# tsurumeso/vocal-remover

Measured on AMD Instinct MI355X. Metric: spectrogram-frames/sec (inference, CascadedNet n_fft=2048), higher is better.
Workload: dtype f32; 1 GPU; configs[1]: 30 s stereo 44.1 kHz synthetic song, STFT -> 11 crops of 256 frames in one device batch -> predict_mask -> stitch -> mask apply -> iSTFT x2; n_fft=2048, hop=1024, cropsize=256, parallelism=replicas x1 (songs shard, no collective), input_residency=inputs resident in HBM when the timed region starts

## Files before the change

__graft_entry__.py:

```python
import concurrent.futures
import importlib.util
import os
import subprocess
import sys

ROOT = os.path.dirname(os.path.abspath(__file__))
PKG_DIR = os.path.join(ROOT, 'vocal-remover_amd')
CSRC = os.path.join(PKG_DIR, 'csrc')
LIB = os.path.join(PKG_DIR, 'libvr_mi355.so')
SOURCES = ['conv_mfma.hip', 'conv_ws.hip', 'conv_dma.hip', 'conv_wino.hip', 'conv_x3.hip', 'conv_x3h.hip', 'conv_x3d.hip', 'conv_x3s.hip', 'conv_thin.hip', 'wgrad_mfma.hip', 'wgrad_wino.hip', 'wgrad_gemm.hip', 'pointwise.hip', 'backward.hip', 'lstm.hip', 'stft.hip', 'augment.hip', 'audio.hip', 'model.hip',
           'train.hip', 'debug.hip', 'comm.hip', 'profile.hip', 'api.cpp', 'pcm_host.cpp']
HEADERS = sorted(f for f in os.listdir(CSRC) if f.endswith('.h')) + [os.path.join('..', '..', 'include', 'vr_mi355.h')]
HIPCC = os.environ.get('HIPCC', '/opt/rocm/bin/hipcc')
FLAGS = ['--offload-arch=gfx950', '-O3', '-std=c++17', '-fPIC', '-Wno-unused-result', '-Rpass-analysis=kernel-resource-usage']
MAX_SCRATCH_BYTES_PER_LANE = 192
ZERO_SCRATCH_KERNELS = ('conv_x3_kernel', 'conv_x3h_kernel', 'conv_x3d_kernel', 'conv_x3d_aspp_kernel', 'wgrad_wino_r_kernel')


def _newer(target, deps):
    if not os.path.exists(target):
        return True
    t = os.path.getmtime(target)
    return any(os.path.getmtime(d) > t for d in deps)


def _compile(src):
    path = os.path.join(CSRC, src)
    obj = os.path.join(CSRC, os.path.splitext(src)[0] + '.o')
    deps = [path] + [os.path.join(CSRC, h) for h in HEADERS]
    if _newer(obj, deps):
        cmd = [HIPCC] + FLAGS + (['-x', 'hip'] if src.endswith('.cpp') else []) + ['-c', path, '-o', obj]
        r = subprocess.run(cmd, capture_output=True, text=True)
        if r.returncode != 0:
# ... 66 lines not shown
```

vocal-remover_amd/csrc/conv_x3d.hip:

```cpp
#include <cstdlib>
#include <type_traits>

#include "conv_epilogue.h"
#include "conv_stage.h"
#include "kernels.h"
#include "lds_dma.h"
#include "x3h_common.h"

namespace vr {

template <int KK, int DH, int DW, int MT, int TH>
struct X3dCfg {
    static_assert(KK == 9 || KK == 1, "3x3 or 1x1");
    static constexpr int TW = 16, CK = 8;
    static constexpr int HH = KK == 9 ? DH : 0, HW = KK == 9 ? DW : 0;
    static constexpr int TH_in = TH + 2 * HH, PW = TW + 2 * HW;
    static constexpr int NSLOT = TH_in * PW;
    static constexpr int NREAL = TH_in * TW;
    static constexpr int NPASS = (NREAL + 255) / 256;
    static constexpr int WM = MT / 32, WN = TH / 8;
    static constexpr int PLANE = NSLOT * 16, P_BYTES = 2 * PLANE;
    static constexpr int NWP = KK * 2 * MT, W_BYTES = NWP * 16, NWPASS = (NWP + 255) / 256;
    static constexpr int E_OFF = P_BYTES + 2 * W_BYTES;
    static constexpr int M_OFF = E_OFF + 4 * MT * 4;
// ... 336 lines not shown
                a.part[((long long)pt * a.Cout + co) * 2 + 1] = s2;
            }
        }
    }
}

__device__ __forceinline__ bool x3d_block(const ConvArgs& a, int& pt, int& ct) {
    const int id = blockIdx.x;
    const int xcd = id & 7, rr = id >> 3;
    ct = rr % a.nct;
    const int per_xcd = (a.npt + 7) >> 3;
    pt = xcd * per_xcd + rr / a.nct;
    return pt < a.npt;
}

template <int KK, int DH, int DW, int MT>
__global__ __launch_bounds__(256, 2) void conv_x3d_kernel(const ConvArgs a) {
    extern __shared__ __attribute__((aligned(16))) char smem_x3d[];
    int pt, ct;
    if (!x3d_block(a, pt, ct)) return;
    x3d_tile<KK, DH, DW, MT, 16>(a, pt, ct, smem_x3d);
}

struct X3dAsppArgs { ConvArgs c[4]; };
template <int MT>
__global__ __launch_bounds__(256, 2) void conv_x3d_aspp_kernel(const X3dAsppArgs g) {
    extern __shared__ __attribute__((aligned(16))) char smem_x3d[];
    int pt, ct;
    if (!x3d_block(g.c[1], pt, ct)) return;
    if (blockIdx.y == 0) x3d_tile<9, 12, 6, MT, 16>(g.c[3], pt, ct, smem_x3d);
    else if (blockIdx.y == 1) x3d_tile<9, 8, 4, MT, 16>(g.c[2], pt, ct, smem_x3d);
    else if (blockIdx.y == 2) x3d_tile<9, 4, 2, MT, 16>(g.c[1], pt, ct, smem_x3d);
    else x3d_tile<1, 1, 1, MT, 16>(g.c[0], pt, ct, smem_x3d);
}

bool x3d_pick(const ConvArgs& a, const ConvShape& s, int* MT_out) {
    static const int enabled = getenv("VR_CONV_X3D") ? atoi(getenv("VR_CONV_X3D")) : 1;
    if (!enabled || a.bf16 != 3 || !a.x3w || a.tapmask) return false;
    if (s.stride != 1 || a.Win != 16 || a.Wout != 16 || a.Hin != a.Hout) return false;
    if (s.KS == 3) {
        const bool dil = (s.dil_h == 1 && s.dil_w == 1) || (s.dil_h == 4 && s.dil_w == 2) || (s.dil_h == 8 && s.dil_w == 4) ||
                         (s.dil_h == 12 && s.dil_w == 6);
        if (!dil || a.pad_h != s.dil_h || a.pad_w != s.dil_w) return false;
    } else if (s.KS == 1) {
        if (a.pad_h != 0 || a.pad_w != 0) return false;
    } else return false;
    for (int i = 0; i < a.nsrc; ++i) {
        const ConvSrc& c = a.src[i];
        if (c.aff0 || c.aff1 || c.post || c.zins || c.up || c.slope != 1.f || c.W != 16 || c.H != a.Hin) return false;
        if ((long long)c.H * (c.sH > 0 ? c.sH : 1) * 4 >= 0x7FFFFFF0LL) return false;
    }
    static const int force_mt = getenv("VR_X3D_MT") ? atoi(getenv("VR_X3D_MT")) : 0;
// ... 20 lines not shown
    VR_HIP(hipGetLastError());
}
template <int MT>
static void x3d_launch_mt(const ConvArgs& a, const ConvShape& s, hipStream_t st) {
    if (s.KS == 1) x3d_launch<1, 1, 1, MT>(a, st);
    else if (s.dil_h == 1) x3d_launch<9, 1, 1, MT>(a, st);
    else if (s.dil_h == 4) x3d_launch<9, 4, 2, MT>(a, st);
    else if (s.dil_h == 8) x3d_launch<9, 8, 4, MT>(a, st);
    else x3d_launch<9, 12, 6, MT>(a, st);
}
void x3d_launch_conv(const ConvArgs& a, const ConvShape& s, int MT, hipStream_t st) {
    if (MT == 64) x3d_launch_mt<64>(a, s, st);
    else x3d_launch_mt<32>(a, s, st);
}

template <int MT>
static void x3d_launch_aspp_mt(const X3dAsppArgs& g, hipStream_t st) {
    auto kern = conv_x3d_aspp_kernel<MT>;
    constexpr int lds = X3dCfg<9, 12, 6, MT, 16>::LDS_BYTES;
    static_assert(lds >= X3dCfg<9, 8, 4, MT, 16>::LDS_BYTES && lds >= X3dCfg<1, 1, 1, MT, 16>::LDS_BYTES, "the widest halo sizes the LDS");
    static std::atomic<unsigned long long> attr_done{0};
    ensure_lds_attr(attr_done, reinterpret_cast<const void*>(kern), lds);
    const ConvArgs& a = g.c[1];
    VR_LAUNCH(kern, dim3((unsigned)((a.npt + 7) / 8 * 8 * a.nct), 4u), dim3(256), lds, st, g);
    VR_HIP(hipGetLastError());
}
bool x3d_aspp_eligible(const ConvArgs* c, const ConvShape* s) {
    static const bool on = !(getenv("VR_ASPP_FUSED") && atoi(getenv("VR_ASPP_FUSED")) == 0);
    if (!on) return false;
    int mt[4];
    for (int j = 0; j < 4; ++j) {
        if (!x3d_pick(c[j], s[j], &mt[j])) return false;
        if (c[j].N != c[0].N || c[j].Hout != c[0].Hout || c[j].CoutPad != c[0].CoutPad) return false;
    }
    return s[0].KS == 1 && s[1].KS == 3 && s[1].dil_h == 4 && s[2].KS == 3 && s[2].dil_h == 8 && s[3].KS == 3 && s[3].dil_h == 12;
}
void x3d_launch_aspp(const ConvArgs* c, hipStream_t st) {
    X3dAsppArgs g;
    int MT = (c[1].CoutPad % 64 == 0) ? 64 : 32;
    if (MT == 64 && (long long)c[1].N * ((c[1].Hout + 15) / 16) * (c[1].CoutPad / 64) * 4 < 512) MT = 32;
    static const int force_mt = getenv("VR_X3D_MT") ? atoi(getenv("VR_X3D_MT")) : 0;
    if ((force_mt == 32 || force_mt == 64) && c[1].CoutPad % force_mt == 0) MT = force_mt;
    for (int j = 0; j < 4; ++j) { g.c[j] = c[j]; x3d_fill_tiling(g.c[j], MT); }
    if (MT == 64) x3d_launch_aspp_mt<64>(g, st);
    else x3d_launch_aspp_mt<32>(g, st);
}

}
```

vocal-remover_amd/csrc/debug.hip:

```cpp
#include <cmath>
#include <cstdlib>
#include <cstring>
#include <memory>
#include <string>
#include <vector>

#include "model.h"

namespace vr {

namespace {

struct DevBuf {
    float* p = nullptr;
    size_t n = 0;
    DevBuf() = default;
    explicit DevBuf(size_t n_) : n(n_) {
        VR_HIP(hipMalloc(&p, (n ? n : 1) * sizeof(float)));
        VR_HIP(hipMemset(p, 0, (n ? n : 1) * sizeof(float)));
        VR_HIP(hipStreamSynchronize(nullptr));
    }
    DevBuf(const float* host, size_t n_) : n(n_) {
        VR_HIP(hipMalloc(&p, (n ? n : 1) * sizeof(float)));
        if (host && n) VR_HIP(hipMemcpy(p, host, n * sizeof(float), hipMemcpyHostToDevice));
// ... 914 lines not shown
        need(5, 0, 2, 1);
        const long long rows = dims[0];
        const int T = (int)dims[1], Wm = (int)dims[2], off = (int)dims[3];
        const bool cplx = dims[4] != 0;
        VR_CHECK(rows > 0 && Wm > 0 && off >= 0 && off + Wm <= T, -2, "crop: need rows, Wm > 0 and 0 <= off, off + Wm <= T");
        const bool loss = !cplx && nin >= 3 && in[2] && nout >= 2 && out[1];
        const size_t E = cplx ? 2 : 1;
        DevBuf m(in[0], (size_t)rows * Wm * E), x(in[1], (size_t)rows * T * E), y(loss ? in[2] : nullptr, loss ? (size_t)rows * T : 0);
        DevBuf part((size_t)l1_crop_blocks()), lossd(4);
        launch_mul_crop(x.p, m.p, cplx, rows, T, Wm, off, st);
        if (loss) launch_l1_crop(L1_CROP_REAL, m.p, y.p, rows, T, Wm, off, part.p, lossd.p, st);
        VR_HIP(hipStreamSynchronize(st));
        m.download(out[0]);
        if (loss) VR_HIP(hipMemcpy(out[1], lossd.p, sizeof(float), hipMemcpyDeviceToHost));
    } else if (name == "rows") {
        need(3, 0, 3, 2);
        const int N = (int)dims[0], R = (int)dims[1], W = (int)dims[2];
        const size_t n = (size_t)N * R * W;
        DevBuf x(in[0], n), aff(in[1], (size_t)R * 2), d(in[2], n), o(n), sums(R);
        launch_rows_affine_relu(x.p, o.p, aff.p, N, R, W, st);
        launch_channel_sum(d.p, N, R, W, sums.p, 0, st);
        VR_HIP(hipStreamSynchronize(st));
        o.download(out[0]); sums.download(out[1]);
    } else if (name == "adam") {
        need(1, 6, 4, 3);
        const size_t n = (size_t)dims[0];
        double dp[6];
        for (int i = 0; i < 6; ++i) {
            char buf[48];
            std::snprintf(buf, sizeof buf, "%.7g", (double)fp[i]);
            dp[i] = std::strtod(buf, nullptr);
        }
        DevBuf p(in[0], n), g(in[1], n), m(in[2], n), v(in[3], n);
        launch_adam(p.p, g.p, m.p, v.p, (long long)n, dp[0], dp[1], dp[2], dp[3], (long long)dp[5], dp[4], st);
        VR_HIP(hipStreamSynchronize(st));
        p.download(out[0]); m.download(out[1]); v.download(out[2]);
    } else if (name == "wire") {
        need(1, 0, 1, 1);
        const size_t n = (size_t)dims[0];
        DevBuf x(in[0], n), half((n + 1) / 2), y(n);
        launch_f32_to_bf16(x.p, reinterpret_cast<unsigned short*>(half.p), (long long)n, st);
        launch_bf16_to_f32(reinterpret_cast<const unsigned short*>(half.p), y.p, (long long)n, st);
        VR_HIP(hipStreamSynchronize(st));
        y.download(out[0]);
    } else if (name == "signal_norm") {
        need(6, 0, 1, 2);
// ... 222 lines not shown
```

vocal-remover_amd/csrc/kernels.h:

```cpp
#pragma once
#include "vr_common.h"

namespace vr {

struct HeadDst {
    float* p;
    long long dN, dC, dH;
    int w_lo, w_hi;
    int pad_rows;
    float* const* items;
    const int* item_pitch;
};
void launch_head_sigmoid(const Tensor& x, const float* w , const HeadDst& d, hipStream_t st);
void launch_head_complex(const Tensor& x, const float* w , const HeadDst& d, hipStream_t st);
int launch_squeeze_conv(const Tensor& x, const float* w , float* out, float* part, bool dry, hipStream_t st,
                        const float* epi = nullptr);

void launch_avgpool_h(const Tensor& x, float* out, hipStream_t st);

struct BNFoldDesc { const float *w, *b, *rm, *rv; float* affine; int C; int bcast; };
void launch_bn_fold_eval(const BNFoldDesc* d_descs, int ndesc, int maxC, float eps, hipStream_t st);
struct BNFinalizeArgs {
    const float* part; int nparts; int pstride;
    double count;
// ... 25 lines not shown
void launch_wino_weights(const float* w, float* u, int Cin, int CoutPad, hipStream_t st);
struct WinoWDesc { const float* w; void* u; int Cin, CoutPad; };
void launch_wino_weights_batched(const WinoWDesc* d_descs, int n, long long max_elems, bool split6, hipStream_t st);
size_t wino_weights6_bytes(int Cin, int CoutPad);
void launch_wino_weights6(const float* w, void* u6, int Cin, int CoutPad, hipStream_t st);
struct X3Tile { int MT, TH; };
struct X3WDesc { const float* w; void* o; int Cin, KK, CoutPad; };
bool x3_pick(const ConvArgs& a, const ConvShape& s, X3Tile* t);
void x3_fill_tiling(ConvArgs& a, const X3Tile& t);
void x3_launch_conv(const ConvArgs& a, const X3Tile& t, hipStream_t st);
size_t x3_weights_bytes(int Cin, int KK, int CoutPad);
void launch_x3_weights(const float* w, void* o, int Cin, int KK, int CoutPad, hipStream_t st);
void launch_x3_weights_batched(const X3WDesc* d_descs, int n, long long max_elems, hipStream_t st);
void x3h_launch_conv(const ConvArgs& a, const X3Tile& t, hipStream_t st);
bool x3h_tail_ok(const ConvArgs& a, const X3Tile& t);
void x3h_trace_read(long long* host, int n);
void x3h_trace_clear();
void launch_x3h_weights(const float* w, void* o, int Cin, int KK, int CoutPad, hipStream_t st);
void launch_x3h_weights_batched(const X3WDesc* d_descs, int n, long long max_elems, int max_cout_pad, hipStream_t st);
bool x3d_pick(const ConvArgs& a, const ConvShape& s, int* MT);
void x3d_fill_tiling(ConvArgs& a, int MT);
void x3d_launch_conv(const ConvArgs& a, const ConvShape& s, int MT, hipStream_t st);
bool x3d_aspp_eligible(const ConvArgs* c4, const ConvShape* s4);
void x3d_launch_aspp(const ConvArgs* c4, hipStream_t st);
bool x3s_pick(const ConvArgs& a, const ConvShape& s, X3Tile* t);
void x3s_fill_tiling(ConvArgs& a, const X3Tile& t);
void x3s_launch_conv(const ConvArgs& a, const X3Tile& t, hipStream_t st);
void launch_upsample2x(const Tensor& x, float* out, hipStream_t st);

void launch_bilstm(const float* gx, const float* whh_f, const float* whh_r, float* out,
                   int N, int T, int H, hipStream_t st);

void launch_bilstm_train(const float* gx, const float* whh_f, const float* whh_r, float* out, float* save,
                         int N, int T, int H, hipStream_t st);
void launch_bilstm_bwd(const float* dh, const float* save, const float* whh_f, const float* whh_r, float* dgx,
                       int N, int T, int H, hipStream_t st);
size_t lstm_whh_grad_scratch_floats(int N, int H);
void launch_lstm_whh_grad(const float* dgx, const float* hout, float* dwhh_f, float* dwhh_r, int N, int T, int H,
                          int accumulate, float* part, hipStream_t st);

struct BnBwdArgs {
    float* g;
    const float* z;
    int N, C, H, W;
    long long sN, sC, sH;
    const float* aff;
    int aff_bcast;
    float slope;
    const float* post;
    const float *gamma, *save_mean, *save_invstd;
    float *dgamma, *dbeta;
    int acc_grads;
    float* coef;
    float* part;
};
int bn_bwd_chunks(const BnBwdArgs& a);
void launch_bn_bwd(const BnBwdArgs& a, hipStream_t st);

void launch_upsample_bwd(const float* dhi, int N, int C, int H, int W, float* glo, long long gN, long long gC,
                         long long gH, int accumulate, hipStream_t st);
void launch_sum_h(const float* d, int N, int C, int H, int W, float* out, hipStream_t st);
void launch_avgpool_bwd(const float* gp, float* g, int N, int C, int H, int W, long long sN, long long sC, long long sH,
// ... 197 lines not shown
```

vocal-remover_amd/csrc/model.h:

```cpp
#pragma once
#include <chrono>
#include <deque>
#include <functional>
#include <map>
#include <memory>
#include <string>
#include <vector>

#include "kernels.h"
#include "weight_forms.h"

namespace vr {

struct Arena {
    char* base = nullptr;
    size_t cap = 0, off = 0, peak = 0;
    bool dry = false;
    void* alloc(size_t bytes) {
        const size_t a = (off + 255) & ~size_t(255);
        off = a + bytes;
        if (off > peak) peak = off;
        if (dry) return reinterpret_cast<void*>(uintptr_t(256));
        if (off > cap) throw Error(-4, "workspace arena overflow (planning bug)");
        return base + a;
// ... 223 lines not shown
    void debug_weight_forms(const float* dw_kmajor, int Cin, int KS, int stride, int dh, int dw, int CoutPad, int Win, bool transformed,
                            ConvArgs& a, LocalConv& lc);
    bool record_taps = false;
    std::map<std::string, Tensor> taps;
    int64_t get_tap(const std::string& name, float* host, int64_t cap_floats, int64_t* shape4);

    bool profiling = false;
    LaunchProfiler* launch_prof = nullptr;
    std::string profile_report;
    void profile_begin();
    void augment_api(const float* Xc, const float* yc, const float* Xi, const float* yi, const void* desc, const float* rw,
                     int B, int T, int bins, bool in_on_dev, float* Xmag, float* ymag, bool out_on_dev, bool out_complex = false);
    void dataset_batch_api(const ResidentSet& set, const ResidentCrop* crops, const void* desc, const float* rw, int B, int T,
                           float* Xmag, float* ymag, bool out_on_dev, bool out_complex = false);
    char* aug_buf = nullptr; size_t aug_cap = 0;
    void aug_reserve(size_t need);
    bool train_wino = true;
    int mfma_mode = 3;
    bool x3_mode() const { return mfma_mode == 2 || mfma_mode == 3; }
    int default_mfma_mode = 3;
    bool serial = false;
    bool crop_window = true;
    bool fuse_tail = true;
    int net_w_lo = 0, net_w_hi = 0;
    void set_option(const std::string& name, int value);
    void reset_adam_state();
    void profile_end(double* conv_ms, double* conv_flops, double* conv_bytes, int* launches);

    hipStream_t stream = nullptr;
    hipStream_t side_stream = nullptr;
    hipEvent_t ev_fork = nullptr, ev_join = nullptr;
    bool band_fork_active = false;
    bool gs_clear_pending = false;
    bool wgrad_on_side = false;
    struct Lane { hipStream_t main = nullptr, side = nullptr; hipEvent_t fork = nullptr, join = nullptr, start = nullptr, done = nullptr; Arena ws; };
    std::vector<Lane> lanes;
    void swap_lane(int i);

private:
    float* p_arena = nullptr; size_t p_floats = 0;
    float* b_arena = nullptr; size_t b_floats = 0;
    Arena ws;
    Arena io;
    void ensure_ws(size_t bytes);
    int plan_B = -1, plan_T = -1; bool plan_training = false; size_t plan_peak = 0;
    void ensure_io(size_t bytes);
// ... 154 lines not shown
```

vocal-remover_amd/csrc/model.hip:

```cpp
#include "pcm.h"
#include "model.h"

#include <algorithm>
#include <chrono>
#include <cmath>
#include <cstdlib>
#include <cstring>

namespace vr {

static inline int round_up(int v, int m) { return (v + m - 1) / m * m; }

Param* Model::add_param(const std::string& key, std::vector<int64_t> shape, ParamKind kind, bool trainable) {
    params.emplace_back();
    Param* p = &params.back();
    p->key = key;
    p->shape = std::move(shape);
    p->kind = kind;
    p->trainable = trainable;
    p->numel = 1;
    for (auto d : p->shape) p->numel *= (size_t)d;
    p->dev_numel = p->numel;
    if (kind == PK_CONV) {
        p->Cout = (int)p->shape[0];
// ... 314 lines not shown
    affine_dirty = false;
}

void Model::set_option(const std::string& name, int value) {
    plan_peak = 0;
    if (name == "train_winograd") train_wino = value != 0;
    else if (name == "serial_exec") serial = value != 0;
    else if (name == "params_dirty") affine_dirty = true;
    else if (name == "mfma_bf16") { mfma_mode = value != 0 ? 1 : default_mfma_mode; affine_dirty = true; }
    else if (name == "mfma_mode") {
        if (value < -1 || value > 3) throw Error(-2, "mfma_mode: 0, 1, 2, 3 or -1 (default)");
        mfma_mode = value < 0 ? default_mfma_mode : value; affine_dirty = true;
    }
    else if (name == "conv_x3d") {
        if (value < -1 || value > 2) throw Error(-2, "conv_x3d: 0, 1, 2 or -1 (default)");
        x3d_mode = value < 0 ? 2 : value;
    }
    else if (name == "conv_x3s") {
        if (value < -1 || value > 1) throw Error(-2, "conv_x3s: 0, 1 or -1 (default)");
        x3s_mode = value < 0 ? x3s_default() : value;
    }
    else if (name == "crop_window") crop_window = value != 0;
    else if (name == "fuse_tail") fuse_tail = value != 0;
    else if (name == "complex_train") {
        if (!is_complex) throw Error(-2, "complex_train: this handle predicts a magnitude mask; the option belongs to complex-mask handles (VR_CREATE_COMPLEX)");
        complex_train = value != 0;
        if (!complex_train && loss_kind != 0) set_loss(0, 0.01);
        graph_valid = false;
    }
    else if (name == "adam_reset") reset_adam_state();
    else if (name == "hip_graph" || name == "conv_x3p" || name == "wgrad_x3h" || name == "conv_x3b") {
        static std::string told;
        if (told.find("|" + name + "|") == std::string::npos) {
            told += "|" + name + "|";
            fprintf(stderr, "libvr_mi355: option '%s' was retired with its kernel (tools/experiments/README.md); ignored\n", name.c_str());
        }
    }
    else throw Error(-2, "unknown option: " + name);
}

void Model::hold_form(FormId f, const std::vector<Conv*>& convs, Wino6Want w6, FormStore& s) {
    if (s.arena[f]) return;
    auto room = [&](const Conv* L) {
        const FormSpec sp = form_spec(f, *L, mfma_mode, w6);
        return sp.held ? (sp.bytes + 255) & ~size_t(255) : size_t(0);
    };
// ... 458 lines not shown
            b->nbt->nbt += 1;
        }
    }
    Tensor zt;
    zt.p = z; zt.N = N; zt.C = nb; zt.H = 1; zt.W = nf;
    zt.sN = (long long)nb * nf; zt.sC = nf; zt.sH = nf;
    if (training) { zt.aff0 = M.squeeze.bn->affine; zt.slope = 0.f; }
    else zt.slope = 1.f;
    if (taping()) {
        zt.g = galloc((size_t)N * nb * nf, false);
        TapeRec r;
        r.kind = TK_SQUEEZE; r.M = &M; r.srcs = {SrcSpec{h}}; r.N = N;
        r.out = zt;
        r.out.C = 1; r.out.H = nb; r.out.sC = (long long)nb * nf; r.out.sH = nf;
        tape.push_back(std::move(r));
    }
    const int G = 4 * M.hid;
    float* bias = ws.allocf((size_t)2 * G);
    if (!training && M.bias_sum) bias = M.bias_sum;
    else if (!dry) {
        launch_add(M.b_ih_f->dev, M.b_hh_f->dev, bias, G, stream);
        launch_add(M.b_ih_r->dev, M.b_hh_r->dev, bias + G, G, stream);
    }
    Tensor gx = run_conv(M.proj, {SrcSpec{zt}}, N, nullptr, bias, true);
    float* hc = ws.allocf((size_t)N * 2 * M.hid * nf);
    float* save = taping() ? ws.allocf((size_t)N * 2 * nf * 5 * M.hid) : nullptr;
    if (!dry) launch_bilstm_train(gx.p, M.whh_f->dev, M.whh_r->dev, hc, save, N, nf, M.hid, stream);
    Tensor ht;
    ht.p = hc; ht.N = N; ht.C = 2 * M.hid; ht.H = 1; ht.W = nf;
    ht.sN = (long long)2 * M.hid * nf; ht.sC = nf; ht.sH = nf; ht.slope = 1.f;
    if (taping()) {
        ht.g = galloc((size_t)N * 2 * M.hid * nf, false);
        TapeRec r;
        r.kind = TK_LSTM; r.M = &M; r.N = N; r.out = ht; r.aux = gx; r.save = save;
        tape.push_back(std::move(r));
    }
    Tensor lin = run_conv(M.dense, {SrcSpec{ht}}, N, nullptr, M.dense_b->dev, true);
    if (taping()) tape.back().bias_param = M.dense_b;
    float* act = training ? ws.allocf((size_t)N * nb * nf) : lin.p;
    if (!dry && training) launch_rows_affine_relu(lin.p, act, M.dense.bn->affine, N, nb, nf, stream);
    Tensor o;
    o.p = act; o.g = lin.g; o.N = N; o.C = 1; o.H = nb; o.W = nf;
    o.sN = (long long)nb * nf; o.sC = (long long)nb * nf; o.sH = nf; o.slope = 1.f;
    return o;
}

Model::SrcSpec Model::upsampled(const Tensor& t) {
    if (training) {
        SrcSpec s{t};
        s.up = true;
        return s;
    }
    static const bool fuse_on = !(getenv("VR_X3_FUSE_UP") && atoi(getenv("VR_X3_FUSE_UP")) == 0);
    static const bool x3_on = !(getenv("VR_CONV_X3") && atoi(getenv("VR_CONV_X3")) == 0);
    if (fuse_on && x3_on && x3_mode() && 4LL * t.H * t.W >= 65536 && 2 * t.W >= 32 && !t.aff0 && !t.aff1 && !t.post && t.slope == 1.f) {
        SrcSpec s{t};
        s.up = true;
        return s;
    }
    Tensor u;
    u.N = t.N; u.C = t.C; u.H = 2 * t.H; u.W = 2 * t.W;
    u.sH = u.W; u.sC = (long long)u.H * u.W; u.sN = u.sC * u.C; u.slope = 1.f;
    u.p = ws.allocf((size_t)u.N * u.C * u.H * u.W);
    if (!dry) launch_upsample2x(t, u.p, stream);
    return SrcSpec{u};
}

Tensor Model::run_basenet(BaseNetL& B, const std::vector<SrcSpec>& in, int N, const Tensor* out_view, FusedTail* tail) {
    const std::string& p = B.prefix;
    Tensor e[5];
    e[0] = run_conv(B.enc1, in, N, nullptr, nullptr, false);
    tap(p + ".e1", e[0]);
    for (int i = 0; i < 4; ++i) {
        Tensor t = run_conv(B.enc_a[i], {SrcSpec{e[i]}}, N, nullptr, nullptr, false);
        e[i + 1] = run_conv(B.enc_b[i], {SrcSpec{t}}, N, nullptr, nullptr, false);
        tap(p + ".e" + std::to_string(i + 2), e[i + 1]);
    }
    const Tensor& x5 = e[4];
    const int C8 = 8 * B.c;
    float* pooled = ws.allocf((size_t)N * C8 * x5.W);
    if (!dry) launch_avgpool_h(x5, pooled, stream);
    Tensor pt;
    pt.p = pooled; pt.N = N; pt.C = C8; pt.H = 1; pt.W = x5.W;
    pt.sN = (long long)C8 * x5.W; pt.sC = x5.W; pt.sH = x5.W; pt.slope = 1.f;
    if (taping()) {
        pt.g = galloc((size_t)N * C8 * x5.W, false);
        TapeRec r;
        r.kind = TK_AVGPOOL; r.srcs = {SrcSpec{x5}}; r.out = pt; r.N = N;
        tape.push_back(std::move(r));
    }
    Tensor f1 = run_conv(B.aspp_pool, {SrcSpec{pt}}, N, nullptr, nullptr, true);
    Tensor cat4;
    cat4.N = N; cat4.C = 4 * C8; cat4.H = x5.H; cat4.W = x5.W;
    cat4.sH = x5.W; cat4.sC = (long long)x5.H * x5.W; cat4.sN = cat4.sC * cat4.C;
    cat4.p = ws.allocf((size_t)N * cat4.C * x5.H * x5.W);
    if (taping()) cat4.g = galloc((size_t)N * cat4.C * x5.H * x5.W, false);
    if (training) { cat4.aff0 = B.aspp_aff; cat4.slope = 0.f; }
    Conv* branch[4] = {&B.aspp_c2, &B.aspp_d[0], &B.aspp_d[1], &B.aspp_d[2]};
    Tensor x5b = x5;
    {
        static const bool mat_enabled = !getenv("VR_NO_TRAIN_MAT");
        if (training && mat_enabled && (x5.aff0 || x5.aff1 || x5.post || x5.slope != 1.f)) {
            float* buf = ws.allocf((size_t)N * C8 * x5.H * x5.W);
            if (!dry) launch_materialize(x5, buf, stream);
            x5b.p = buf; x5b.aff0 = x5b.aff1 = nullptr; x5b.post = nullptr; x5b.slope = 1.f; x5b.hsplit = 1 << 30;
            x5b.sH = x5.W; x5b.sC = (long long)x5.H * x5.W; x5b.sN = x5b.sC * C8;
        }
    }
    static const bool aspp_fork = !getenv("VR_NO_ASPP_FORK");
    std::vector<PendingConv> pend;
    const bool group = !dry && mfma_mode == 3 && x3d_mode == 2 && !(training && !train_wino);
    const bool afk = aspp_fork && !serial && !training && !dry && !profiling && side_stream != nullptr && !band_fork_active && !group;
    hipStream_t aspp_main = stream;
    if (afk) {
        hipEvent_t ef = ev_fork;
        VR_HIP(hipEventRecord(ef, aspp_main));
        VR_HIP(hipStreamWaitEvent(side_stream, ef, 0));
    }
    for (int j = 0; j < 4; ++j) {
        Tensor v = cat4;
        v.C = C8;
        v.p = dry ? cat4.p : cat4.p + (long long)j * C8 * cat4.sC;
        if (taping() && !dry) v.g = cat4.g + (long long)j * C8 * cat4.sC;
        if (afk) stream = (j & 1) ? side_stream : aspp_main;
        if (group) conv_sink = &pend;
        try { run_conv(*branch[j], {SrcSpec{x5b}}, N, &v, nullptr, false); } catch (...) { stream = aspp_main; conv_sink = nullptr; throw; }
        conv_sink = nullptr;
    }
    if (group) {
        VR_CHECK(pend.size() == 4, -3, "ASPP: four branch convs expected");
        ConvArgs c4[4];
        ConvShape s4[4];
        double flops = 0.0, bytes = 0.0;
        for (int j = 0; j < 4; ++j) { c4[j] = pend[j].a; s4[j] = pend[j].shp; flops += pend[j].flops; bytes += pend[j].bytes; }
        if (x3d_aspp_eligible(c4, s4)) {
            record_begin(0, flops);
            if (profiling) {
                char tag[160];
                snprintf(tag, sizeof tag, "%s.aspp.conv2-5 k1+3x(k3 d4/8/12) ci%d co%d %dx%dx%d", p.c_str(), C8, C8, N, x5.H, x5.W);
                record_note(bytes - 3.0 * 4.0 * (double)N * C8 * x5.H * x5.W, tag);
            }
            x3d_launch_aspp(c4, stream);
            record_end();
        } else {
            for (int j = 0; j < 4; ++j) {
                record_begin(0, pend[j].flops);
                if (profiling) record_note(pend[j].bytes, branch[j]->name.c_str());
                launch_conv(c4[j], s4[j], stream);
                record_end();
            }
        }
        for (int j = 0; j < 4; ++j)
            if (pend[j].stats) {
                launch_bn_finalize(pend[j].fin, stream);
                pend[j].bn->nbt->nbt += 1;
            }
    }
    if (afk) {
        stream = aspp_main;
        hipEvent_t ej = ev_join;
        VR_HIP(hipEventRecord(ej, side_stream));
        VR_HIP(hipStreamWaitEvent(aspp_main, ej, 0));
    }
    SrcSpec s1{f1};
    s1.bcastH = x5.H;
// ... 1268 lines not shown
```

Before: 191,000 spectrogram-frames/sec.

## Fuse ASPP pooled branch into grouped launch and add split-K rows GEMM for LSTM

The ASPP pooled branch (height average-pool plus 1x1 conv) now runs as an extra grid slice inside the grouped dilated-conv launch, so it no longer needs separate pool and conv launches. Separately, the BiLSTM input projection and dense layer use a new MFMA rows-GEMM kernel with split-K across waves and an LDS reduction, replacing the general conv path at inference. Both target launch overhead and poor utilisation on small, thin matrix products. The fused pool slice runs on one block per sample per cout tile and may sit on the critical path, and the new GEMM adds a code path that has to match the conv numerics.

```diff
diff --git a/__graft_entry__.py b/__graft_entry__.py
--- a/__graft_entry__.py
+++ b/__graft_entry__.py
@@ -8,7 +8,7 @@
 PKG_DIR = os.path.join(ROOT, 'vocal-remover_amd')
 CSRC = os.path.join(PKG_DIR, 'csrc')
 LIB = os.path.join(PKG_DIR, 'libvr_mi355.so')
-SOURCES = ['conv_mfma.hip', 'conv_ws.hip', 'conv_dma.hip', 'conv_wino.hip', 'conv_x3.hip', 'conv_x3h.hip', 'conv_x3d.hip', 'conv_x3s.hip', 'conv_thin.hip', 'wgrad_mfma.hip', 'wgrad_wino.hip', 'wgrad_gemm.hip', 'pointwise.hip', 'backward.hip', 'lstm.hip', 'stft.hip', 'augment.hip', 'audio.hip', 'model.hip',
+SOURCES = ['conv_mfma.hip', 'conv_ws.hip', 'conv_dma.hip', 'conv_wino.hip', 'conv_x3.hip', 'conv_x3h.hip', 'conv_x3d.hip', 'conv_x3s.hip', 'conv_thin.hip', 'wgrad_mfma.hip', 'wgrad_wino.hip', 'wgrad_gemm.hip', 'pointwise.hip', 'backward.hip', 'lstm.hip', 'rows_gemm.hip', 'stft.hip', 'augment.hip', 'audio.hip', 'model.hip',
            'train.hip', 'debug.hip', 'comm.hip', 'profile.hip', 'api.cpp', 'pcm_host.cpp']
 HEADERS = sorted(f for f in os.listdir(CSRC) if f.endswith('.h')) + [os.path.join('..', '..', 'include', 'vr_mi355.h')]
 HIPCC = os.environ.get('HIPCC', '/opt/rocm/bin/hipcc')
diff --git a/vocal-remover_amd/csrc/conv_x3d.hip b/vocal-remover_amd/csrc/conv_x3d.hip
--- a/vocal-remover_amd/csrc/conv_x3d.hip
+++ b/vocal-remover_amd/csrc/conv_x3d.hip
@@ -382,12 +382,72 @@
     x3d_tile<KK, DH, DW, MT, 16>(a, pt, ct, smem_x3d);
 }
 
-struct X3dAsppArgs { ConvArgs c[4]; };
+template <int MT>
+__device__ __forceinline__ void x3d_pool_tile(const X3dPoolArgs& q, const int n, const int ct, char* const smem) {
+    float* const pooled = reinterpret_cast<float*>(smem);
+    const int tid = threadIdx.x;
+    const float* const xn = q.x + (long long)n * q.xN;
+    const float rows = (float)q.H;
+    for (int i = tid; i < q.C8 * 4; i += 256) {
+        const float* xc = xn + (long long)(i >> 2) * q.xC + (i & 3) * 4;
+        vr_f32x4h s = {0.f, 0.f, 0.f, 0.f};
+        int h = 0;
+        for (; h + 8 <= q.H; h += 8) {
+            vr_f32x4h v[8];
+#pragma unroll
+            for (int j = 0; j < 8; ++j) v[j] = *reinterpret_cast<const vr_f32x4h*>(xc + (long long)(h + j) * q.xH);
+#pragma unroll
+            for (int j = 0; j < 8; ++j) s += v[j];
+        }
+        for (; h < q.H; ++h) s += *reinterpret_cast<const vr_f32x4h*>(xc + (long long)h * q.xH);
+        *reinterpret_cast<vr_f32x4h*>(pooled + i * 4) = s / rows;
+    }
+    __syncthreads();
+    constexpr int CPT = MT / 16;
+    const int w = tid & 15;
+    const int co = ct * MT + (tid >> 4) * CPT;
+    const float* wp = q.w + co;
+    float acc[CPT];
+#pragma unroll
+    for (int j = 0; j < CPT; ++j) acc[j] = 0.f;
+#pragma unroll 16
+    for (int ci = 0; ci < q.C8; ++ci) {
+        const float p = pooled[ci * 16 + w];
+        float wv[CPT];
+        if (CPT == 4) {
+            const vr_f32x4h v = *reinterpret_cast<const vr_f32x4h*>(wp + (long long)ci * q.CoutPad);
+#pragma unroll
+            for (int j = 0; j < CPT; ++j) wv[j] = v[j];
+        } else {
+            const vr_f32x2 v = *reinterpret_cast<const vr_f32x2*>(wp + (long long)ci * q.CoutPad);
+#pragma unroll
+            for (int j = 0; j < CPT; ++j) wv[j] = v[j];
+        }
+#pragma unroll
+        for (int j = 0; j < CPT; ++j) acc[j] = fmaf(wv[j], p, acc[j]);
+    }
+#pragma unroll
+    for (int j = 0; j < CPT; ++j) {
+        const int c = co + j;
+        if (c < q.Cout) {
+            float v = acc[j];
+            if (q.epi) v = act_apply(fmaf(v, q.epi[2 * c], q.epi[2 * c + 1]), q.slope);
+            q.out[((long long)n * q.Cout + c) * 16 + w] = v;
+        }
+    }
+}
+
+struct X3dAsppArgs { ConvArgs c[4]; X3dPoolArgs pool; };
 template <int MT>
 __global__ __launch_bounds__(256, 2) void conv_x3d_aspp_kernel(const X3dAsppArgs g) {
     extern __shared__ __attribute__((aligned(16))) char smem_x3d[];
     int pt, ct;
     if (!x3d_block(g.c[1], pt, ct)) return;
+    if (blockIdx.y == 4) {
+        const int n = pt / g.c[1].tiles_h;
+        if (pt - n * g.c[1].tiles_h == 0) x3d_pool_tile<MT>(g.pool, n, ct, smem_x3d);
+        return;
+    }
     if (blockIdx.y == 0) x3d_tile<9, 12, 6, MT, 16>(g.c[3], pt, ct, smem_x3d);
     else if (blockIdx.y == 1) x3d_tile<9, 8, 4, MT, 16>(g.c[2], pt, ct, smem_x3d);
     else if (blockIdx.y == 2) x3d_tile<9, 4, 2, MT, 16>(g.c[1], pt, ct, smem_x3d);
@@ -454,7 +514,7 @@
     static std::atomic<unsigned long long> attr_done{0};
     ensure_lds_attr(attr_done, reinterpret_cast<const void*>(kern), lds);
     const ConvArgs& a = g.c[1];
-    VR_LAUNCH(kern, dim3((unsigned)((a.npt + 7) / 8 * 8 * a.nct), 4u), dim3(256), lds, st, g);
+    VR_LAUNCH(kern, dim3((unsigned)((a.npt + 7) / 8 * 8 * a.nct), g.pool.x ? 5u : 4u), dim3(256), lds, st, g);
     VR_HIP(hipGetLastError());
 }
 bool x3d_aspp_eligible(const ConvArgs* c, const ConvShape* s) {
@@ -467,8 +527,19 @@
     }
     return s[0].KS == 1 && s[1].KS == 3 && s[1].dil_h == 4 && s[2].KS == 3 && s[2].dil_h == 8 && s[3].KS == 3 && s[3].dil_h == 12;
 }
-void x3d_launch_aspp(const ConvArgs* c, hipStream_t st) {
+bool x3d_pool_eligible(const X3dPoolArgs& q, const ConvArgs* c) {
+    if (!q.x || !q.w || !q.out || q.C8 < 1 || q.H < 1 || q.Cout < 1) return false;
+    if (q.CoutPad != c[1].CoutPad || q.CoutPad % 32 != 0 || q.Cout > q.CoutPad || q.H != c[1].Hin || c[1].Win != 16) return false;
+    if (((size_t)q.x & 15) || (q.xN & 3) || (q.xC & 3) || (q.xH & 3)) return false;
+    return (long long)q.C8 * 16 * 4 <= X3dCfg<9, 12, 6, 32, 16>::LDS_BYTES;
+}
+void x3d_launch_aspp(const ConvArgs* c, hipStream_t st, const X3dPoolArgs* pool) {
     X3dAsppArgs g;
+    g.pool = X3dPoolArgs{};
+    if (pool) {
+        VR_CHECK(x3d_pool_eligible(*pool, c), -3, "conv_x3d: the ASPP group launch cannot carry this pooled branch");
+        g.pool = *pool;
+    }
     int MT = (c[1].CoutPad % 64 == 0) ? 64 : 32;
     if (MT == 64 && (long long)c[1].N * ((c[1].Hout + 15) / 16) * (c[1].CoutPad / 64) * 4 < 512) MT = 32;
     static const int force_mt = getenv("VR_X3D_MT") ? atoi(getenv("VR_X3D_MT")) : 0;
diff --git a/vocal-remover_amd/csrc/debug.hip b/vocal-remover_amd/csrc/debug.hip
--- a/vocal-remover_amd/csrc/debug.hip
+++ b/vocal-remover_amd/csrc/debug.hip
@@ -960,6 +960,100 @@
         launch_channel_sum(d.p, N, R, W, sums.p, 0, st);
         VR_HIP(hipStreamSynchronize(st));
         o.download(out[0]); sums.download(out[1]);
+    } else if (name == "rows_gemm") {
+        need(6, 1, 2, 1);
+        const int N = (int)dims[0], T = (int)dims[1], K = (int)dims[2], Cout = (int)dims[3], CoutPad = (int)dims[4];
+        const bool conv_too = dims[5] & 1;
+        VR_CHECK(N >= 1 && T >= 1 && K >= 1 && Cout >= 1 && CoutPad >= 1 && in[0] && in[1] && out[0], -2, "rows_gemm: sizes must be positive");
+        VR_CHECK(!conv_too || (nout >= 2 && out[1] && CoutPad % 32 == 0 && CoutPad >= Cout), -2, "rows_gemm: the conv launch needs couts padded to 32 and out[1]");
+        const size_t no = (size_t)N * Cout * T;
+        DevBuf x(in[0], (size_t)N * K * T), w(in[1], (size_t)K * CoutPad);
+        DevBuf bias(nin >= 3 ? in[2] : nullptr, nin >= 3 && in[2] ? (size_t)Cout : 0), epi(nin >= 4 ? in[3] : nullptr, nin >= 4 && in[3] ? (size_t)Cout * 2 : 0);
+        const bool has_bias = nin >= 3 && in[2], has_epi = nin >= 4 && in[3];
+        GuardedBuf o(out[0], no);
+        RowsGemmArgs g{};
+        g.x = x.p; g.xN = (long long)K * T; g.w = w.p; g.bias = has_bias ? bias.p : nullptr; g.epi = has_epi ? epi.p : nullptr; g.slope = fp[0];
+        g.out = o.p(); g.N = N; g.T = T; g.K = K; g.Cout = Cout; g.CoutPad = CoutPad;
+        launch_rows_gemm(g, st, ndims >= 7 ? (int)dims[6] : 0);
+        DevBuf oc(conv_too ? no : 0);
+        if (conv_too) {
+            ConvArgs a{};
+            a.nsrc = 1; a.N = 1; a.Cin = K; a.c1 = a.c2 = K; a.Cout = Cout; a.CoutPad = CoutPad;
+            a.d1 = a.d2 = 1 << 30;
+            a.bf16 = mfma_mode;
+            Tensor xt = dense(x.p, N, K, 1, T);
+            a.src[0] = make_src(xt, false, 0);
+            a.src[0].sH = a.src[0].sN; a.src[0].sN = 0; a.src[0].H = N;
+            a.Hin = a.Hout = N; a.Win = a.Wout = T;
+            a.w = w.p; a.bias = g.bias;
+            if (has_epi) { a.epi = epi.p; a.epi_slope = fp[0]; }
+            a.dst[0] = ConvDst{oc.p, 0, (long long)T, (long long)Cout * T, 0, 0};
+            launch_conv(a, ConvShape{1, 1, 1, 1}, st);
+        }
+        VR_HIP(hipStreamSynchronize(st));
+        VR_CHECK(o.intact(), -3, "rows_gemm: a store outside the output buffer");
+        o.download(out[0]);
+        if (conv_too) oc.download(out[1]);
+    } else if (name == "aspp_pool") {
+        need(3, 1, 8, 4);
+        const int N = (int)dims[0], C8 = (int)dims[1], H = (int)dims[2], W = 16, CoutPad = (C8 + 31) / 32 * 32;
+        VR_CHECK(N >= 1 && C8 >= 1 && H >= 1, -2, "aspp_pool: sizes must be positive");
+        VR_CHECK(mfma_mode == 3, -2, "aspp_pool: the group launch runs in mfma_mode 3");
+        for (int i = 0; i < 8; ++i) VR_CHECK(in[i] != nullptr, -2, "aspp_pool: missing input");
+        const size_t nx = (size_t)N * C8 * H * W, nf = (size_t)N * C8 * W;
+        DevBuf x(in[0], nx), epi1(in[2], (size_t)C8 * 2), epib(in[7], (size_t)4 * C8 * 2), cat_a(4 * nx), cat_b(4 * nx), pooled(nf), f1b(nf);
+        GuardedBuf f1a(out[0], nf);
+        const Tensor xt = dense(x.p, N, C8, H, W);
+        std::vector<std::unique_ptr<DevBuf>> keep;
+        auto kmajor = [&](const float* oihw, int KK) {
+            std::vector<float> wk((size_t)C8 * KK * CoutPad, 0.f);
+            for (int co = 0; co < C8; ++co)
+                for (int ci = 0; ci < C8; ++ci)
+                    for (int k = 0; k < KK; ++k) wk[((size_t)ci * KK + k) * CoutPad + co] = oihw[((size_t)co * C8 + ci) * KK + k];
+            keep.emplace_back(new DevBuf(wk.data(), wk.size()));
+            return keep.back()->p;
+        };
+        ConvArgs c4[4];
+        ConvShape s4[4];
+        LocalConv wf[4];
+        for (int j = 0; j < 4; ++j) {
+            const int KS = j ? 3 : 1, dh = j ? 4 * j : 1, dw = j ? 2 * j : 1;
+            ConvArgs& a = c4[j];
+            a = ConvArgs{};
+            a.nsrc = 1; a.src[0] = make_src(xt, false, 0); a.c1 = a.c2 = a.Cin = C8;
+            a.w = kmajor(in[3 + j], KS * KS); a.Cout = C8; a.CoutPad = CoutPad;
+            a.epi = epib.p + (size_t)j * C8 * 2; a.epi_slope = 0.f;
+            a.bf16 = 3; a.d1 = a.d2 = 1 << 30;
+            a.N = N; a.Hin = a.Hout = H; a.Win = a.Wout = W; a.pad_h = j ? dh : 0; a.pad_w = j ? dw : 0;
+            debug_weight_forms(a.w, C8, KS, 1, dh, dw, CoutPad, W, true, a, wf[j]);
+            a.dst[0] = ConvDst{cat_a.p + (size_t)j * C8 * H * W, (long long)4 * C8 * H * W, (long long)H * W, W, 0, 0};
+            s4[j] = ConvShape{KS, 1, dh, dw};
+        }
+        VR_CHECK(x3d_aspp_eligible(c4, s4), -2, "aspp_pool: conv_x3d does not take these four branch convs as one launch");
+        X3dPoolArgs q{};
+        q.x = x.p; q.xN = xt.sN; q.xC = xt.sC; q.xH = xt.sH;
+        q.w = kmajor(in[1], 1); q.epi = epi1.p; q.slope = fp[0]; q.out = f1a.p();
+        q.C8 = C8; q.H = H; q.Cout = C8; q.CoutPad = CoutPad;
+        VR_CHECK(x3d_pool_eligible(q, c4), -2, "aspp_pool: the group launch cannot carry this pooled branch (x3d_pool_eligible)");
+        x3d_launch_aspp(c4, st, &q);
+        for (int j = 0; j < 4; ++j) c4[j].dst[0].p = cat_b.p + (size_t)j * C8 * H * W;
+        launch_avgpool_h(xt, pooled.p, st);
+        {
+            ConvArgs b{};
+            b.nsrc = 1; b.N = 1; b.Cin = C8; b.c1 = b.c2 = C8; b.Cout = C8; b.CoutPad = CoutPad;
+            b.d1 = b.d2 = 1 << 30;
+            b.bf16 = 3;
+            b.src[0] = make_src(dense(pooled.p, N, C8, 1, W), false, 0);
+            b.src[0].sH = b.src[0].sN; b.src[0].sN = 0; b.src[0].H = N;
+            b.Hin = b.Hout = N; b.Win = b.Wout = W;
+            b.w = q.w; b.epi = epi1.p; b.epi_slope = fp[0];
+            b.dst[0] = ConvDst{f1b.p, 0, (long long)W, (long long)C8 * W, 0, 0};
+            launch_conv(b, ConvShape{1, 1, 1, 1}, st);
+        }
+        x3d_launch_aspp(c4, st);
+        VR_HIP(hipStreamSynchronize(st));
+        VR_CHECK(f1a.intact(), -3, "aspp_pool: a store outside f1's buffer");
+        f1a.download(out[0]); cat_a.download(out[1]); f1b.download(out[2]); cat_b.download(out[3]);
     } else if (name == "adam") {
         need(1, 6, 4, 3);
         const size_t n = (size_t)dims[0];
diff --git a/vocal-remover_amd/csrc/kernels.h b/vocal-remover_amd/csrc/kernels.h
--- a/vocal-remover_amd/csrc/kernels.h
+++ b/vocal-remover_amd/csrc/kernels.h
@@ -71,7 +71,17 @@
 void x3d_fill_tiling(ConvArgs& a, int MT);
 void x3d_launch_conv(const ConvArgs& a, const ConvShape& s, int MT, hipStream_t st);
 bool x3d_aspp_eligible(const ConvArgs* c4, const ConvShape* s4);
-void x3d_launch_aspp(const ConvArgs* c4, hipStream_t st);
+struct X3dPoolArgs {
+    const float* x;
+    long long xN, xC, xH;
+    const float* w;
+    const float* epi;
+    float slope;
+    float* out;
+    int C8, H, Cout, CoutPad;
+};
+bool x3d_pool_eligible(const X3dPoolArgs& q, const ConvArgs* c4);
+void x3d_launch_aspp(const ConvArgs* c4, hipStream_t st, const X3dPoolArgs* pool = nullptr);
 bool x3s_pick(const ConvArgs& a, const ConvShape& s, X3Tile* t);
 void x3s_fill_tiling(ConvArgs& a, const X3Tile& t);
 void x3s_launch_conv(const ConvArgs& a, const X3Tile& t, hipStream_t st);
@@ -87,6 +97,20 @@
 size_t lstm_whh_grad_scratch_floats(int N, int H);
 void launch_lstm_whh_grad(const float* dgx, const float* hout, float* dwhh_f, float* dwhh_r, int N, int T, int H,
                           int accumulate, float* part, hipStream_t st);
+
+struct RowsGemmArgs {
+    const float* x;
+    long long xN;
+    const float* w;
+    const float* bias;
+    const float* epi;
+    float slope;
+    float* out;
+    int N, T, K, Cout, CoutPad;
+};
+bool rows_gemm_ok(const RowsGemmArgs& a);
+int rows_gemm_tile(const RowsGemmArgs& a);
+void launch_rows_gemm(const RowsGemmArgs& a, hipStream_t st, int tile = 0);
 
 struct BnBwdArgs {
     float* g;
diff --git a/vocal-remover_amd/csrc/model.h b/vocal-remover_amd/csrc/model.h
--- a/vocal-remover_amd/csrc/model.h
+++ b/vocal-remover_amd/csrc/model.h
@@ -269,6 +269,8 @@
     bool serial = false;
     bool crop_window = true;
     bool fuse_tail = true;
+    bool lstm_gemm = true;
+    bool aspp_pool_fused = true;
     int net_w_lo = 0, net_w_hi = 0;
     void set_option(const std::string& name, int value);
     void reset_adam_state();
diff --git a/vocal-remover_amd/csrc/model.hip b/vocal-remover_amd/csrc/model.hip
--- a/vocal-remover_amd/csrc/model.hip
+++ b/vocal-remover_amd/csrc/model.hip
@@ -360,6 +360,8 @@
     }
     else if (name == "crop_window") crop_window = value != 0;
     else if (name == "fuse_tail") fuse_tail = value != 0;
+    else if (name == "lstm_gemm") lstm_gemm = value != 0;
+    else if (name == "aspp_pool_fused") aspp_pool_fused = value != 0;
     else if (name == "complex_train") {
         if (!is_complex) throw Error(-2, "complex_train: this handle predicts a magnitude mask; the option belongs to complex-mask handles (VR_CREATE_COMPLEX)");
         complex_train = value != 0;
@@ -864,7 +866,28 @@
         launch_add(M.b_ih_f->dev, M.b_hh_f->dev, bias, G, stream);
         launch_add(M.b_ih_r->dev, M.b_hh_r->dev, bias + G, G, stream);
     }
-    Tensor gx = run_conv(M.proj, {SrcSpec{zt}}, N, nullptr, bias, true);
+    const bool gemm = lstm_gemm && !training && !taping() && !conv_sink;
+    auto rows_gemm = [&](Conv& L, const Tensor& x, const float* b) {
+        Tensor o;
+        o.N = N; o.C = L.Cout; o.H = 1; o.W = nf;
+        o.p = ws.allocf((size_t)N * L.Cout * nf); o.sN = (long long)L.Cout * nf; o.sC = nf; o.sH = nf; o.slope = 1.f;
+        if (dry) return o;
+        RowsGemmArgs g{};
+        g.x = x.p; g.xN = x.sN; g.w = L.w->dev; g.bias = b; g.out = o.p;
+        if (L.bn) { g.epi = L.bn->affine; g.slope = L.slope; }
+        g.N = N; g.T = nf; g.K = L.Cin; g.Cout = L.Cout; g.CoutPad = L.CoutPad;
+        VR_CHECK(L.KS == 1 && x.C == L.Cin && x.sC == nf && rows_gemm_ok(g), -3, "rows_gemm: " + L.name + " is not a matrix product it takes");
+        record_begin(0, 2.0 * N * (double)nf * L.Cout * L.Cin);
+        if (profiling) {
+            char tag[160];
+            snprintf(tag, sizeof tag, "%s gemm ci%d co%d 1x%dx%d", L.name.c_str(), L.Cin, L.Cout, N, nf);
+            record_note(4.0 * ((double)N * L.Cin * nf + (double)N * L.Cout * nf + (double)L.Cin * L.Cout), tag);
+        }
+        launch_rows_gemm(g, stream);
+        record_end();
+        return o;
+    };
+    Tensor gx = gemm ? rows_gemm(M.proj, zt, bias) : run_conv(M.proj, {SrcSpec{zt}}, N, nullptr, bias, true);
     float* hc = ws.allocf((size_t)N * 2 * M.hid * nf);
     float* save = taping() ? ws.allocf((size_t)N * 2 * nf * 5 * M.hid) : nullptr;
     if (!dry) launch_bilstm_train(gx.p, M.whh_f->dev, M.whh_r->dev, hc, save, N, nf, M.hid, stream);
@@ -877,7 +900,7 @@
         r.kind = TK_LSTM; r.M = &M; r.N = N; r.out = ht; r.aux = gx; r.save = save;
         tape.push_back(std::move(r));
     }
-    Tensor lin = run_conv(M.dense, {SrcSpec{ht}}, N, nullptr, M.dense_b->dev, true);
+    Tensor lin = gemm ? rows_gemm(M.dense, ht, M.dense_b->dev) : run_conv(M.dense, {SrcSpec{ht}}, N, nullptr, M.dense_b->dev, true);
     if (taping()) tape.back().bias_param = M.dense_b;
     float* act = training ? ws.allocf((size_t)N * nb * nf) : lin.p;
     if (!dry && training) launch_rows_affine_relu(lin.p, act, M.dense.bn->affine, N, nb, nf, stream);
@@ -921,7 +944,9 @@
     const Tensor& x5 = e[4];
     const int C8 = 8 * B.c;
     float* pooled = ws.allocf((size_t)N * C8 * x5.W);
-    if (!dry) launch_avgpool_h(x5, pooled, stream);
+    const bool group = !dry && mfma_mode == 3 && x3d_mode == 2 && !(training && !train_wino);
+    const bool pool_wait = group && !training && aspp_pool_fused;
+    if (!dry && !pool_wait) launch_avgpool_h(x5, pooled, stream);
     Tensor pt;
     pt.p = pooled; pt.N = N; pt.C = C8; pt.H = 1; pt.W = x5.W;
     pt.sN = (long long)C8 * x5.W; pt.sC = x5.W; pt.sH = x5.W; pt.slope = 1.f;
@@ -931,7 +956,11 @@
         r.kind = TK_AVGPOOL; r.srcs = {SrcSpec{x5}}; r.out = pt; r.N = N;
         tape.push_back(std::move(r));
     }
-    Tensor f1 = run_conv(B.aspp_pool, {SrcSpec{pt}}, N, nullptr, nullptr, true);
+    std::vector<PendingConv> pend_pool;
+    if (pool_wait) conv_sink = &pend_pool;
+    Tensor f1;
+    try { f1 = run_conv(B.aspp_pool, {SrcSpec{pt}}, N, nullptr, nullptr, true); } catch (...) { conv_sink = nullptr; throw; }
+    conv_sink = nullptr;
     Tensor cat4;
     cat4.N = N; cat4.C = 4 * C8; cat4.H = x5.H; cat4.W = x5.W;
     cat4.sH = x5.W; cat4.sC = (long long)x5.H * x5.W; cat4.sN = cat4.sC * cat4.C;
@@ -951,7 +980,6 @@
     }
     static const bool aspp_fork = !getenv("VR_NO_ASPP_FORK");
     std::vector<PendingConv> pend;
-    const bool group = !dry && mfma_mode == 3 && x3d_mode == 2 && !(training && !train_wino);
     const bool afk = aspp_fork && !serial && !training && !dry && !profiling && side_stream != nullptr && !band_fork_active && !group;
     hipStream_t aspp_main = stream;
     if (afk) {
@@ -975,14 +1003,36 @@
         ConvShape s4[4];
         double flops = 0.0, bytes = 0.0;
         for (int j = 0; j < 4; ++j) { c4[j] = pend[j].a; s4[j] = pend[j].shp; flops += pend[j].flops; bytes += pend[j].bytes; }
-        if (x3d_aspp_eligible(c4, s4)) {
-            record_begin(0, flops);
+        const bool grouped = x3d_aspp_eligible(c4, s4);
+        X3dPoolArgs q{};
+        if (pool_wait) {
+            VR_CHECK(pend_pool.size() == 1, -3, "ASPP: the pooled branch's conv expected");
+            const ConvArgs& pa = pend_pool[0].a;
+            const ConvSrc& xs = c4[0].src[0];
+            q.x = xs.p; q.xN = xs.sN; q.xC = xs.sC; q.xH = xs.sH;
+            q.w = pa.w; q.epi = pa.epi; q.slope = pa.epi ? pa.epi_slope : 1.f; q.out = f1.p;
+            q.C8 = C8; q.H = x5.H; q.Cout = pa.Cout; q.CoutPad = pa.CoutPad;
+        }
+        const bool pool_in = pool_wait && grouped && c4[0].nsrc == 1 && !pend_pool[0].a.bias && f1.sN == (long long)q.Cout * 16 && f1.sC == 16 &&
+                             x3d_pool_eligible(q, c4);
+        if (pool_wait && !pool_in) {
+            launch_avgpool_h(x5, pooled, stream);
+            record_begin(0, pend_pool[0].flops);
+            if (profiling) record_note(pend_pool[0].bytes, B.aspp_pool.name.c_str());
+            launch_conv(pend_pool[0].a, pend_pool[0].shp, stream);
+            record_end();
+        }
+        if (grouped) {
+            const double pflops = pool_in ? (double)N * C8 * x5.H * x5.W + pend_pool[0].flops : 0.0;
+            const double pbytes = pool_in ? 4.0 * ((double)C8 * C8 + (double)N * C8 * x5.W) : 0.0;
+            record_begin(0, flops + pflops);
             if (profiling) {
                 char tag[160];
-                snprintf(tag, sizeof tag, "%s.aspp.conv2-5 k1+3x(k3 d4/8/12) ci%d co%d %dx%dx%d", p.c_str(), C8, C8, N, x5.H, x5.W);
-                record_note(bytes - 3.0 * 4.0 * (double)N * C8 * x5.H * x5.W, tag);
+                snprintf(tag, sizeof tag, "%s.aspp.conv2-5%s k1+3x(k3 d4/8/12) ci%d co%d %dx%dx%d", p.c_str(), pool_in ? "+pool+conv1" : "", C8, C8, N,
+                         x5.H, x5.W);
+                record_note(bytes - 3.0 * 4.0 * (double)N * C8 * x5.H * x5.W + pbytes, tag);
             }
-            x3d_launch_aspp(c4, stream);
+            x3d_launch_aspp(c4, stream, pool_in ? &q : nullptr);
             record_end();
         } else {
             for (int j = 0; j < 4; ++j) {
diff --git a/vocal-remover_amd/csrc/rows_gemm.hip b/vocal-remover_amd/csrc/rows_gemm.hip
--- /dev/null
+++ b/vocal-remover_amd/csrc/rows_gemm.hip
@@ -0,0 +1,136 @@
+#include "conv_stage.h"
+#include "kernels.h"
+
+namespace vr {
+
+typedef float rg_f32x4 __attribute__((ext_vector_type(4)));
+
+__device__ __forceinline__ float rg_keep(float v, bool keep) { return __uint_as_float(__float_as_uint(v) & (keep ? 0xFFFFFFFFu : 0u)); }
+
+template <int MC, int NP>
+__global__ __launch_bounds__(256) void rows_gemm_kernel(const RowsGemmArgs a) {
+    constexpr int NB = 16;
+    constexpr int NS = MC * NP;
+    __shared__ float red[4][NS][4][64];
+    const int tid = threadIdx.x;
+    const int lane = tid & 63;
+    const int wave = __builtin_amdgcn_readfirstlane(tid >> 6);
+    const int l16 = lane & 15, kq = lane >> 4;
+    const int P = a.N * a.T;
+    const int co0 = blockIdx.y * (16 * MC), p0 = blockIdx.x * (16 * NP);
+    const float* wb[MC];
+    bool cok[MC];
+#pragma unroll
+    for (int mc = 0; mc < MC; ++mc) {
+        const int co = co0 + 16 * mc + l16;
+        cok[mc] = co < a.Cout;
+        wb[mc] = a.w + (cok[mc] ? co : a.Cout - 1);
+    }
+    const float* xb[NP];
+    bool pok[NP];
+    long long ob[NP];
+#pragma unroll
+    for (int np = 0; np < NP; ++np) {
+        const int p = p0 + 16 * np + l16;
+        pok[np] = p < P;
+        const int pc = pok[np] ? p : P - 1;
+        const int n = pc / a.T, t = pc - n * a.T;
+        xb[np] = a.x + (long long)n * a.xN + t;
+        ob[np] = (long long)n * a.Cout * a.T + t;
+    }
+
+    const int nsteps = (a.K + 3) >> 2;
+    const int per = (nsteps + 3) >> 2;
+    const int sbeg = wave * per;
+    const int send = min(sbeg + per, nsteps);
+
+    rg_f32x4 acc[MC][NP];
+#pragma unroll
+    for (int mc = 0; mc < MC; ++mc)
+#pragma unroll
+        for (int np = 0; np < NP; ++np) acc[mc][np] = rg_f32x4{0.f, 0.f, 0.f, 0.f};
+    for (int s0 = sbeg; s0 < send; s0 += NB) {
+        float av[MC][NB], bv[NP][NB];
+#pragma unroll
+        for (int i = 0; i < NB; ++i) {
+            const int k = (s0 + i) * 4 + kq;
+            const int kc = s0 + i < send && k < a.K ? k : a.K - 1;
+#pragma unroll
+            for (int mc = 0; mc < MC; ++mc) av[mc][i] = wb[mc][(long long)kc * a.CoutPad];
+#pragma unroll
+            for (int np = 0; np < NP; ++np) bv[np][i] = xb[np][(long long)kc * a.T];
+        }
+        __builtin_amdgcn_sched_barrier(0);
+#pragma unroll
+        for (int i = 0; i < NB; ++i) {
+            const bool kok = s0 + i < send && (s0 + i) * 4 + kq < a.K;
+            float am[MC], bm[NP];
+#pragma unroll
+            for (int mc = 0; mc < MC; ++mc) am[mc] = rg_keep(av[mc][i], kok && cok[mc]);
+#pragma unroll
+            for (int np = 0; np < NP; ++np) bm[np] = rg_keep(bv[np][i], kok && pok[np]);
+#pragma unroll
+            for (int mc = 0; mc < MC; ++mc)
+#pragma unroll
+                for (int np = 0; np < NP; ++np) acc[mc][np] = __builtin_amdgcn_mfma_f32_16x16x4f32(am[mc], bm[np], acc[mc][np], 0, 0, 0);
+        }
+    }
+#pragma unroll
+    for (int mc = 0; mc < MC; ++mc)
+#pragma unroll
+        for (int np = 0; np < NP; ++np)
+#pragma unroll
+            for (int r = 0; r < 4; ++r) red[wave][mc * NP + np][r][lane] = acc[mc][np][r];
+    __syncthreads();
+#pragma unroll
+    for (int mc = 0; mc < MC; ++mc)
+#pragma unroll
+        for (int np = 0; np < NP; ++np) {
+            const int j = mc * NP + np;
+            if ((j & 3) != wave) continue;
+#pragma unroll
+            for (int r = 0; r < 4; ++r) {
+                const int c = co0 + 16 * mc + 4 * kq + r;
+                float v = ((red[0][j][r][lane] + red[1][j][r][lane]) + red[2][j][r][lane]) + red[3][j][r][lane];
+                if (c < a.Cout && pok[np]) {
+                    if (a.bias) v += a.bias[c];
+                    if (a.epi) v = act_apply(fmaf(v, a.epi[2 * c], a.epi[2 * c + 1]), a.slope);
+                    a.out[ob[np] + (long long)c * a.T] = v;
+                }
+            }
+        }
+}
+
+bool rows_gemm_ok(const RowsGemmArgs& a) {
+    if (!a.x || !a.w || !a.out) return false;
+    if (a.N < 1 || a.T < 1 || a.K < 1 || a.Cout < 1 || a.CoutPad < a.Cout) return false;
+    if ((long long)a.N * a.T > 0x7FFFFFF0LL / 16 || a.xN < (long long)a.K * a.T) return false;
+    return (a.Cout + 15) / 16 <= 65535;
+}
+
+int rows_gemm_tile(const RowsGemmArgs& a) {
+    const long long P = (long long)a.N * a.T;
+    auto groups = [&](int mc, int np) { return ((P + 16 * np - 1) / (16 * np)) * ((a.Cout + 16 * mc - 1) / (16 * mc)); };
+    if (groups(2, 2) >= 512) return 22;
+    if (groups(2, 1) >= 512) return 21;
+    return 11;
+}
+
+template <int MC, int NP>
+static void rows_gemm_launch(const RowsGemmArgs& a, hipStream_t st) {
+    const int P = a.N * a.T;
+    VR_LAUNCH((rows_gemm_kernel<MC, NP>), dim3((unsigned)((P + 16 * NP - 1) / (16 * NP)), (unsigned)((a.Cout + 16 * MC - 1) / (16 * MC))), dim3(256),
+              0, st, a);
+    VR_HIP(hipGetLastError());
+}
+
+void launch_rows_gemm(const RowsGemmArgs& a, hipStream_t st, int tile) {
+    VR_CHECK(rows_gemm_ok(a), -2, "rows_gemm: N, T, K, Cout >= 1, CoutPad >= Cout, a sample pitch of at least K T, at most 65535 cout tiles");
+    if (!tile) tile = rows_gemm_tile(a);
+    VR_CHECK(tile == 11 || tile == 21 || tile == 22, -2, "rows_gemm: tiles are 11 (16 couts x 16 positions), 21 (32 x 16) and 22 (32 x 32)");
+    if (tile == 22) rows_gemm_launch<2, 2>(a, st);
+    else if (tile == 21) rows_gemm_launch<2, 1>(a, st);
+    else rows_gemm_launch<1, 1>(a, st);
+}
+
+}
```

Measured after the change: 194,000 spectrogram-frames/sec (median of 6 runs). +1.6%, better.
